# ShawnHuang497/MedPLIB

Measured on AMD Instinct MI355X. Metric: train samples/sec (img+64tok), higher is better.
Workload: dtype bf16

## Files before the change

### medplib_amd/csrc/gemm320_bf16.hip

```cpp
#include "gemm_common.h"
#include <stdlib.h>
#include <algorithm>

namespace {

constexpr int BM3 = 320, BN3 = 256, BK3 = 64, NT3 = 512;
constexpr int A_BYTES = BM3 * 128, B_BYTES = BN3 * 128, STAGE3 = A_BYTES + B_BYTES;

__device__ __forceinline__ int lds_off3(int r, int c) { return r * 128 + ((c ^ (r & 7)) << 4); }

#define MP3_BAR()                          \
  do {                                     \
    asm volatile("" ::: "memory");         \
    __builtin_amdgcn_sched_barrier(0);     \
    __builtin_amdgcn_s_barrier();          \
    __builtin_amdgcn_sched_barrier(0);     \
    asm volatile("" ::: "memory");         \
  } while (0)
#define MP3_LGKM0() asm volatile("s_waitcnt lgkmcnt(0)" ::: "memory")

constexpr int EPI_PLAIN = 0, EPI_ROPE = 1, EPI_SWIGLU = 2, EPI_COMBINE = 3, EPI_RELU = 4, EPI_GELU = 5;
template <int EPI>
__device__ __forceinline__ void gemm320_epilogue(const GemmArgs& g, f32x4 (&acc)[5][8], int batch, int M, int N, int m0, int n0, int wr, int wc,
                                                 int fr, int fq, unsigned items = 0xfffffu) {
  bf16_t* Cb = reinterpret_cast<bf16_t*>(g.C) + batch * g.sC;
  const int cw = n0 + wc * 128;
  const int c8 = pair_col8(fq);
  if constexpr (EPI == EPI_SWIGLU) {
    float rsc[5] = {1.f, 1.f, 1.f, 1.f, 1.f};
    if (g.a_scale) {
#pragma unroll
      for (int i = 0; i < 5; ++i) {
        const int row = m0 + wr * 80 + i * 16 + fr;
        if (row < M) rsc[i] = g.a_scale[g.a_rows ? g.a_rows[batch * g.rows_stride + row] : row];
      }
    }
#pragma unroll
    for (int i = 0; i < 5; ++i) {
      const int row = m0 + wr * 80 + i * 16 + fr;
#pragma unroll
      for (int jb = 0; jb < 2; ++jb) {
        if (!((items >> (i * 4 + jb * 2)) & 1u)) continue;
        bf16x4 o[2];
#pragma unroll
        for (int jj = 0; jj < 2; ++jj)
#pragma unroll
          for (int r = 0; r < 4; ++r) {
            acc[i][jb * 4 + jj][r] *= rsc[i];
            acc[i][jb * 4 + jj + 2][r] *= rsc[i];
            const float gf = (float)(bf16_t)acc[i][jb * 4 + jj][r];
            const float uf = (float)(bf16_t)acc[i][jb * 4 + jj + 2][r];
            o[jj][r] = (bf16_t)(gf * mp_sigmoid_fast(gf) * uf);
          }
        const bf16x8 p = pair_swap16(o[0], o[1]);
        if (row < M) *reinterpret_cast<bf16x8*>(Cb + (int64_t)row * g.ldc + (cw >> 1) + jb * 32 + c8) = p;
        if (g.keep_gu) {
          const bf16x8 pg = pair_swap16(round4(acc[i][jb * 4]), round4(acc[i][jb * 4 + 1])), pu = pair_swap16(round4(acc[i][jb * 4 + 2]), round4(acc[i][jb * 4 + 3]));
          if (row < M) {
            *reinterpret_cast<bf16x8*>(g.keep_gu + (int64_t)row * g.ld_gu + cw + jb * 64 + c8) = pg;
            *reinterpret_cast<bf16x8*>(g.keep_gu + (int64_t)row * g.ld_gu + cw + jb * 64 + 32 + c8) = pu;
          }
        }
      }
      __builtin_amdgcn_sched_barrier(0);
    }
    return;
  }
  if constexpr (EPI == EPI_COMBINE) {
    bf16_t* Cs = reinterpret_cast<bf16_t*>(g.C);
    int orow[5];
    float sc[5];
#pragma unroll
    for (int i = 0; i < 5; ++i) {
      const int row = m0 + wr * 80 + i * 16 + fr;
      orow[i] = row < M ? g.c_rows[batch * g.rows_stride + row] : -1;
    }
#pragma unroll
    for (int i = 0; i < 5; ++i) sc[i] = (orow[i] >= 0 && g.c_scale) ? g.c_scale[orow[i]] : 1.f;
#pragma unroll
    for (int h = 0; h < 2; ++h) {
      bf16x8 rv[5][2];
#pragma unroll
      for (int i = 0; i < 5; ++i)
#pragma unroll
        for (int jp = 0; jp < 2; ++jp) {
          const int col = cw + (h * 2 + jp) * 32 + c8;
          rv[i][jp] = bf16x8{};
          if (g.residual && orow[i] >= 0 && ((items >> (i * 4 + h * 2 + jp)) & 1u))
            rv[i][jp] = *reinterpret_cast<const bf16x8*>(g.residual + (int64_t)orow[i] * g.ldr + col);
        }
      __builtin_amdgcn_sched_barrier(0);
#pragma unroll
      for (int i = 0; i < 5; ++i)
#pragma unroll
        for (int jp = 0; jp < 2; ++jp) {
          const int col = cw + (h * 2 + jp) * 32 + c8;
          const bf16x8 p = pair_swap16(round4(acc[i][(h * 2 + jp) * 2]), round4(acc[i][(h * 2 + jp) * 2 + 1]));
          bf16x8 o;
#pragma unroll
          for (int e = 0; e < 8; ++e) {
            float v = (float)p[e] * sc[i];
            if (g.residual) v += (float)rv[i][jp][e];
            o[e] = (bf16_t)v;
          }
          if (orow[i] >= 0 && ((items >> (i * 4 + h * 2 + jp)) & 1u)) *reinterpret_cast<bf16x8*>(Cs + (int64_t)orow[i] * g.ldc + col) = o;
        }
      __builtin_amdgcn_sched_barrier(0);
    }
    return;
  }
  if constexpr (EPI == EPI_ROPE) {
    const bool is_v = n0 >= (N / 3) * 2;
    const int head0 = (cw >> 7) << 7;
    f32x4 cs[2][2][2], sn[2][2][2];
    float rsc[2] = {1.f, 1.f};
    auto fetch = [&](int i, int buf) {
      const int row = m0 + wr * 80 + i * 16 + fr;
      const int pos = (row < M ? row : 0) % g.rope_seq + g.rope_pos0;
      if (g.a_scale) rsc[buf] = g.a_scale[row < M ? row : 0];
#pragma unroll
      for (int jb = 0; jb < 2; ++jb)
#pragma unroll
        for (int jj = 0; jj < 2; ++jj) {
          const int dim = jb * 32 + jj * 16 + fq * 4;
          cs[buf][jb][jj] = *reinterpret_cast<const f32x4*>(g.rope_cos + (int64_t)pos * 64 + dim);
          sn[buf][jb][jj] = *reinterpret_cast<const f32x4*>(g.rope_sin + (int64_t)pos * 64 + dim);
        }
    };
    fetch(0, 0);
#pragma unroll
    for (int i = 0; i < 5; ++i) {
      if (i + 1 < 5) fetch(i + 1, (i + 1) & 1);
      __builtin_amdgcn_sched_barrier(0);
      const int row = m0 + wr * 80 + i * 16 + fr;
#pragma unroll
      for (int jb = 0; jb < 2; ++jb) {
        bf16x4 olo[2], ohi[2];
#pragma unroll
        for (int jj = 0; jj < 2; ++jj) {
          const bf16x4 qa = round4(acc[i][jb * 4 + jj] * rsc[i & 1]), qb = round4(acc[i][jb * 4 + jj + 2] * rsc[i & 1]);
#pragma unroll
          for (int r = 0; r < 4; ++r) {
            const float a = (float)qa[r], b = (float)qb[r];
            const bf16_t rlo = (bf16_t)(a * cs[i & 1][jb][jj][r] - b * sn[i & 1][jb][jj][r]);
            const bf16_t rhi = (bf16_t)(b * cs[i & 1][jb][jj][r] + a * sn[i & 1][jb][jj][r]);
            olo[jj][r] = is_v ? qa[r] : rlo;
            ohi[jj][r] = is_v ? qb[r] : rhi;
          }
        }
        const bf16x8 plo = pair_swap16(olo[0], olo[1]), phi = pair_swap16(ohi[0], ohi[1]);
        const int col_lo = (is_v ? cw + jb * 64 : head0 + jb * 32) + c8;
        const int col_hi = (is_v ? cw + jb * 64 + 32 : head0 + 64 + jb * 32) + c8;
        if (row < M) {
          *reinterpret_cast<bf16x8*>(Cb + (int64_t)row * g.ldc + col_lo) = plo;
          *reinterpret_cast<bf16x8*>(Cb + (int64_t)row * g.ldc + col_hi) = phi;
        }
      }
      __builtin_amdgcn_sched_barrier(0);
    }
    return;
  }
  const float* bias0 = g.bias ? g.bias + batch * g.sBias : nullptr;
  if (g.alpha != 1.f || bias0) {
#pragma unroll
    for (int j = 0; j < 8; ++j) {
      f32x4 bv = {0.f, 0.f, 0.f, 0.f};
      if (bias0) {
#pragma unroll
        for (int r = 0; r < 4; ++r) { const int col = cw + j * 16 + fq * 4 + r; bv[r] = col < N ? bias0[col] : 0.f; }
      }
#pragma unroll
      for (int i = 0; i < 5; ++i) acc[i][j] = acc[i][j] * g.alpha + bv;
    }
  }
#define MP3_ACT_SWEEP(EXPR)                                                          \
  _Pragma("unroll") for (int i = 0; i < 5; ++i) _Pragma("unroll") for (int j = 0; j < 8; ++j) {                    \
    _Pragma("unroll") for (int r = 0; r < 4; ++r) { const float v = acc[i][j][r]; acc[i][j][r] = (EXPR); }         \
    __builtin_amdgcn_sched_barrier(0);                                                                             \
  }
  if constexpr (EPI == EPI_RELU) { MP3_ACT_SWEEP(fmaxf(v, 0.f)) }
  else if constexpr (EPI == EPI_GELU) { MP3_ACT_SWEEP(gelu_erf_fast(v)) }
  else if (g.act == ACT_QUICK_GELU) { MP3_ACT_SWEEP(v * mp_sigmoid_fast(v, 1.702f)) }
#undef MP3_ACT_SWEEP
  const bf16_t* R = g.residual ? g.residual + batch * g.sR : nullptr;
#pragma unroll
  for (int h = 0; h < 2; ++h) {
    bf16x8 rv[5][2];
    if (R) {
#pragma unroll
      for (int i = 0; i < 5; ++i) {
        const int row = m0 + wr * 80 + i * 16 + fr;
#pragma unroll
        for (int jp = 0; jp < 2; ++jp) {
          const int col = cw + (h * 2 + jp) * 32 + c8;
          rv[i][jp] = bf16x8{};
          if (row < M && col < N && ((items >> (i * 4 + h * 2 + jp)) & 1u)) rv[i][jp] = *reinterpret_cast<const bf16x8*>(R + (int64_t)row * g.ldr + col);
        }
      }
      __builtin_amdgcn_sched_barrier(0);
    }
#pragma unroll
    for (int i = 0; i < 5; ++i) {
      const int row = m0 + wr * 80 + i * 16 + fr;
#pragma unroll
      for (int jp = 0; jp < 2; ++jp) {
        const int col = cw + (h * 2 + jp) * 32 + c8;
        bf16x8 p = pair_swap16(round4(acc[i][(h * 2 + jp) * 2]), round4(acc[i][(h * 2 + jp) * 2 + 1]));
        if (R) {
#pragma unroll
          for (int e = 0; e < 8; ++e) p[e] = (bf16_t)((float)p[e] + (float)rv[i][jp][e]);
        }
        if (row < M && col < N && ((items >> (i * 4 + h * 2 + jp)) & 1u)) *reinterpret_cast<bf16x8*>(Cb + (int64_t)row * g.ldc + col) = p;
      }
    }
    __builtin_amdgcn_sched_barrier(0);
  }
}

constexpr int MAX_FLAT_BATCH3 = 8;
template <int EPI>
__global__ __launch_bounds__(NT3, 1) void gemm320_bf16_nt_kernel(GemmArgs g) {
  extern __shared__ __attribute__((aligned(16))) char smem[];
  const int N = g.N;
  const int tiles_n = N / BN3;
  int T = 0;
  int pre[MAX_FLAT_BATCH3];
#pragma unroll
  for (int b = 0; b < MAX_FLAT_BATCH3; ++b) {
    pre[b] = T;
    if (b < g.nbatch) {
      const int Mb = g.m_dev ? min(g.M, g.m_dev[b * g.m_dev_stride]) : g.M;
      T += ((Mb + BM3 - 1) / BM3) * tiles_n;
    }
  }
  const int C = g.n_cu;
  const int full = (T / C) * C, rem = T - full;
  const int nt_all = g.K / BK3;
  int S = 1;
  if (g.ws && rem > 0 && rem * 2 <= C) S = max(1, min(min(min(C / rem, g.max_split), nt_all / 4), EPI == EPI_SWIGLU ? 10 : 20));
  const int bid = blockIdx.x;
  if (bid >= full + rem * S) return;
  int flat, split = 0;
  if (bid < full) {
    flat = (bid & 7) * (full >> 3) + (bid >> 3);
  } else {
    const int r = bid - full;
    if (S == 1 && (rem & 7) == 0) {
      flat = full + (r & 7) * (rem >> 3) + (r >> 3);
    } else {
      flat = full + r % rem;
      split = r / rem;
    }
  }
  const bool is_split = (bid >= full) && S > 1;
  int batch = 0, pbase = 0;
#pragma unroll
  for (int b = 1; b < MAX_FLAT_BATCH3; ++b) if (b < g.nbatch && flat >= pre[b]) { batch = b; pbase = pre[b]; }
  const int lid = flat - pbase;
  const int M = g.m_dev ? min(g.M, g.m_dev[batch * g.m_dev_stride]) : g.M;
  const int tiles_m = (M + BM3 - 1) / BM3;
  const int GROUP_M = g.group_m;
  const int per_group = GROUP_M * tiles_n;
  const int grp = lid / per_group;
  const int first_m = grp * GROUP_M;
  const int gsz = min(tiles_m - first_m, GROUP_M);
  const int tm = first_m + (lid % per_group) % gsz, tn = (lid % per_group) / gsz;
  const int m0 = tm * BM3, n0 = tn * BN3;
  int kt0 = 0, nt = nt_all;
  if (is_split) {
    const int base = nt_all / S, extra = nt_all % S;
    kt0 = split * base + min(split, extra);
    nt = base + (split < extra ? 1 : 0);
  }
  const int k_byte0 = kt0 * (BK3 * 2);

  const int tid = threadIdx.x;
  const int lane = tid & 63;
  const int wave = __builtin_amdgcn_readfirstlane(tid >> 6);
  const int wc = wave >> 2, wr = wave & 3;
  const int fr = lane & 15, fq = lane >> 4;

  const int sub_row = lane >> 3;
  const int src_c = (lane & 7) ^ sub_row;
  const __amdgpu_buffer_rsrc_t rs_a = __builtin_amdgcn_make_buffer_rsrc(const_cast<bf16_t*>(g.A + batch * g.sA), 0,
                                          g.a_rows ? 0x7ffffff0 : (int)(((int64_t)(M - 1) * g.lda + g.K) * 2), 0x00020000);
  const __amdgpu_buffer_rsrc_t rs_w = __builtin_amdgcn_make_buffer_rsrc(const_cast<bf16_t*>(g.W + batch * g.sW), 0, (int)(((int64_t)(N - 1) * g.ldw + g.K) * 2), 0x00020000);
  const int w_lane = (int)((sub_row * g.ldw + src_c * 8) * 2);
  const int w_row_bytes = (int)(g.ldw * 2);
  int a_off[5];
#pragma unroll
  for (int i = 0; i < 5; ++i) {
    int row = m0 + (wave + 8 * i) * 8 + sub_row;
    if (g.a_rows) row = g.a_rows[batch * g.rows_stride + min(row, M - 1)];
    a_off[i] = (int)(((int64_t)row * g.lda + src_c * 8) * 2);
  }
  int b_piece[4];
#pragma unroll
  for (int k = 0; k < 4; ++k) {
    const int e = 2 * wave + (k & 1);
    b_piece[k] = (e & 7) + (e >> 3) * 16 + (k >> 1) * 8;
  }
  auto dma_a = [&](int i, int t) {
    __builtin_amdgcn_raw_ptr_buffer_load_lds(rs_a, (__attribute__((address_space(3))) void*)(smem + (t & 1) * STAGE3 + (wave + 8 * i) * 1024), 16,
                                             a_off[i], k_byte0 + t * (BK3 * 2), 0, 0);
  };
  auto dma_b = [&](int k, int t) {
    __builtin_amdgcn_raw_ptr_buffer_load_lds(rs_w, (__attribute__((address_space(3))) void*)(smem + (t & 1) * STAGE3 + A_BYTES + b_piece[k] * 1024), 16,
                                             w_lane, (n0 + b_piece[k] * 8) * w_row_bytes + k_byte0 + t * (BK3 * 2), 0, 0);
  };

  f32x4 acc[5][8];
#pragma unroll
  for (int i = 0; i < 5; ++i)
#pragma unroll
    for (int j = 0; j < 8; ++j) acc[i][j] = f32x4{0.f, 0.f, 0.f, 0.f};
  bf16x8 fa[5][2], fb[4][2];
  const int a_rd0 = (wr * 80 + fr) * 128 + ((fq ^ (fr & 7)) << 4), a_rd1 = (wr * 80 + fr) * 128 + (((4 + fq) ^ (fr & 7)) << 4);
  const int b_rd0 = A_BYTES + (wc * 128 + fr) * 128 + ((fq ^ (fr & 7)) << 4), b_rd1 = A_BYTES + (wc * 128 + fr) * 128 + (((4 + fq) ^ (fr & 7)) << 4);
  auto load_a = [&](const char* st) {
#pragma unroll
    for (int i = 0; i < 5; ++i) {
      fa[i][0] = *reinterpret_cast<const bf16x8*>(st + a_rd0 + i * 2048);
      fa[i][1] = *reinterpret_cast<const bf16x8*>(st + a_rd1 + i * 2048);
    }
  };
  auto load_b = [&](int hn, const char* st) {
#pragma unroll
    for (int j = 0; j < 4; ++j) {
      fb[j][0] = *reinterpret_cast<const bf16x8*>(st + b_rd0 + (hn * 64 + j * 16) * 128);
      fb[j][1] = *reinterpret_cast<const bf16x8*>(st + b_rd1 + (hn * 64 + j * 16) * 128);
    }
  };
#ifndef MP3_PRIO
#define MP3_PRIO 0
#endif
#define MP3_MFMA_40(HN)                                                                                     \
  do {                                                                                                      \
    if (MP3_PRIO == 0) __builtin_amdgcn_s_setprio(1);                                                       \
    _Pragma("unroll") for (int kk = 0; kk < 2; ++kk)                                                        \
      _Pragma("unroll") for (int i = 0; i < 5; ++i)                                                         \
        _Pragma("unroll") for (int j = 0; j < 4; ++j)                                                       \
          acc[i][(HN) * 4 + j] = __builtin_amdgcn_mfma_f32_16x16x32_bf16(fb[j][kk], fa[i][kk], acc[i][(HN) * 4 + j], 0, 0, 0); \
    if (MP3_PRIO == 0) __builtin_amdgcn_s_setprio(0);                                                       \
    MP3_BAR();                                                                                              \
  } while (0)

#pragma unroll
  for (int i = 0; i < 5; ++i) dma_a(i, 0);
#pragma unroll
  for (int k = 0; k < 4; ++k) dma_b(k, 0);
  if (nt > 1) {
#pragma unroll
    for (int i = 0; i < 5; ++i) dma_a(i, 1);
    dma_b(0, 1); dma_b(1, 1);
    asm volatile("s_waitcnt vmcnt(7)" ::: "memory");
  } else {
    asm volatile("s_waitcnt vmcnt(0)" ::: "memory");
  }
  MP3_BAR();
  if (wc == 1) MP3_BAR();
  if (MP3_PRIO == 2 && wc == 1) __builtin_amdgcn_s_setprio(1);

  for (int t = 0; t < nt; ++t) {
    const char* st = smem + (t & 1) * STAGE3;
    const bool n1 = (t + 1 < nt), n2 = (t + 2 < nt);
    load_b(0, st);
    load_a(st);
    __builtin_amdgcn_sched_barrier(0);
    if (n1) { dma_b(2, t + 1); dma_b(3, t + 1); }
    MP3_LGKM0();
    MP3_BAR();
    MP3_MFMA_40(0);
    load_b(1, st);
    __builtin_amdgcn_sched_barrier(0);
    if (n2) {
#pragma unroll
      for (int i = 0; i < 5; ++i) dma_a(i, t + 2);
      dma_b(0, t + 2); dma_b(1, t + 2);
      asm volatile("s_waitcnt vmcnt(7)" ::: "memory");
    } else {
      asm volatile("s_waitcnt vmcnt(0)" ::: "memory");
    }
    MP3_LGKM0();
    MP3_BAR();
    MP3_MFMA_40(1);
  }
  if (wc == 0) MP3_BAR();
  if (MP3_PRIO == 2) __builtin_amdgcn_s_setprio(0);
  unsigned items = 0xfffffu;
  if (is_split) {
    typedef __attribute__((ext_vector_type(4))) unsigned int u32x4;
    constexpr int SLAB = BM3 * BN3 * 4;
    const int tail = flat - full;
    float* tile_ws = g.ws + ((int64_t)tail * S) * (BM3 * BN3);
    const __amdgpu_buffer_rsrc_t rs = __builtin_amdgcn_make_buffer_rsrc(tile_ws, 0, S * SLAB, 0x00020000);
    const int my_off = split * SLAB + tid * 16;
#pragma unroll
    for (int i = 0; i < 5; ++i)
#pragma unroll
      for (int j = 0; j < 8; ++j)
        __builtin_amdgcn_raw_buffer_store_b128(__builtin_bit_cast(u32x4, acc[i][j]), rs, my_off + (i * 8 + j) * (NT3 * 16), 0, 16);
    asm volatile("s_waitcnt vmcnt(0)" ::: "memory");
    __syncthreads();
    int* arrive = g.tickets + tail;
    int* depart = g.tickets + 128 + tail;
    int* mode = g.tickets + 256 + tail;
    constexpr int MODE_COOP = 1, MODE_LAST = 2;
    int* s_flag = reinterpret_cast<int*>(smem);
    if (tid == 0) {
      __hip_atomic_fetch_add(arrive, 1, __ATOMIC_RELAXED, __HIP_MEMORY_SCOPE_AGENT);
      const long long t0 = __builtin_amdgcn_s_memtime();
      int m = 0, seen = 0;
      for (;;) {
        seen = __hip_atomic_load(arrive, __ATOMIC_RELAXED, __HIP_MEMORY_SCOPE_AGENT);
        if (seen >= S) break;
        m = __hip_atomic_load(mode, __ATOMIC_RELAXED, __HIP_MEMORY_SCOPE_AGENT);
        if (m) break;
        if (__builtin_amdgcn_s_memtime() - t0 > g.tail_wait) break;
        __builtin_amdgcn_s_sleep(8);
      }
      if (!m) {
        int expected = 0;
        const int want = seen >= S ? MODE_COOP : MODE_LAST;
        m = __hip_atomic_compare_exchange_strong(mode, &expected, want, __ATOMIC_RELAXED, __ATOMIC_RELAXED, __HIP_MEMORY_SCOPE_AGENT) ? want : expected;
      }
      int last = 0;
      if (m == MODE_LAST) last = __hip_atomic_fetch_add(depart, 1, __ATOMIC_RELAXED, __HIP_MEMORY_SCOPE_AGENT) == S - 1;
      s_flag[0] = m | (last << 8);
    }
    __syncthreads();
    const int decided = s_flag[0];
    __syncthreads();
    const bool coop = (decided & 0xff) == MODE_COOP;
    if (!coop && !(decided >> 8)) return;
    constexpr int N_ITEMS = (EPI == EPI_SWIGLU) ? 10 : 20;
    items = 0;
#pragma unroll
    for (int it = 0; it < N_ITEMS; ++it)
      if (!coop || it % S == split) items |= (EPI == EPI_SWIGLU) ? (3u << (2 * it)) : (1u << it);
#pragma unroll
    for (int i = 0; i < 5; ++i)
#pragma unroll
      for (int j = 0; j < 8; ++j) acc[i][j] = f32x4{0.f, 0.f, 0.f, 0.f};
    for (int sp = 0; sp < S; ++sp) {
      const int base = sp * SLAB + tid * 16;
#pragma unroll
      for (int it = 0; it < 20; ++it) {
        if (!((items >> it) & 1u)) continue;
        const int i = it >> 2, j0 = (it & 3) * 2;
        u32x4 t[2];
#pragma unroll
        for (int q = 0; q < 2; ++q) t[q] = __builtin_amdgcn_raw_buffer_load_b128(rs, base + (i * 8 + j0 + q) * (NT3 * 16), 0, 16);
#pragma unroll
        for (int q = 0; q < 2; ++q) acc[i][j0 + q] += __builtin_bit_cast(f32x4, t[q]);
      }
    }
    asm volatile("s_waitcnt vmcnt(0)" ::: "memory");
    __syncthreads();
    if (tid == 0) {
      const bool rearm = coop ? (__hip_atomic_fetch_add(depart, 1, __ATOMIC_RELAXED, __HIP_MEMORY_SCOPE_AGENT) == S - 1) : true;
      if (rearm) {
        __hip_atomic_store(depart, 0, __ATOMIC_RELAXED, __HIP_MEMORY_SCOPE_AGENT);
        __hip_atomic_store(mode, 0, __ATOMIC_RELAXED, __HIP_MEMORY_SCOPE_AGENT);
        __hip_atomic_store(arrive, 0, __ATOMIC_RELAXED, __HIP_MEMORY_SCOPE_AGENT);
      }
    }
  }
  int tid2 = threadIdx.x;
  asm volatile("" : "+v"(tid2));
  gemm320_epilogue<EPI>(g, acc, batch, M, N, m0, n0, (tid2 >> 6) & 3, tid2 >> 8, tid2 & 15, (tid2 >> 4) & 3, items);
}

}

bool mp_gemm320_eligible(const GemmArgs& g, int batch) {
  if (batch < 1 || batch > MAX_FLAT_BATCH3 || g.out_f32) return false;
  if (g.keep_gu && (batch != 1 || (g.ld_gu & 7) || (reinterpret_cast<uintptr_t>(g.keep_gu) & 15))) return false;
  if (!(g.act == ACT_NONE || g.act == ACT_QUICK_GELU || g.act == ACT_ROPE_QK || g.act == ACT_SWIGLU_PAIR || g.act == ACT_RELU || g.act == ACT_GELU)) return false;
  if ((g.act == ACT_RELU || g.act == ACT_GELU) && (g.c_rows || g.a_rows)) return false;
  if (g.act == ACT_ROPE_QK && (batch != 1 || g.m_dev || g.a_rows || g.c_rows)) return false;
  if (g.act == ACT_SWIGLU_PAIR && (g.c_rows || g.residual || g.bias || g.alpha != 1.f || ((g.N >> 1) & 7))) return false;
  if (g.c_rows && (g.act != ACT_NONE || g.bias || g.alpha != 1.f)) return false;
  if (g.a_scale && !(g.act == ACT_ROPE_QK || g.act == ACT_SWIGLU_PAIR)) return false;
  if (g.N % BN3 || g.K % BK3 || g.M < (mp_gemm_policy_whole_tiles() ? BM3 : 1024)) return false;
  if ((g.ldc & 7) || (reinterpret_cast<uintptr_t>(g.C) & 15) || (g.sC & 7)) return false;
  if (g.residual && ((g.ldr & 7) || (reinterpret_cast<uintptr_t>(g.residual) & 15) || (g.sR & 7))) return false;
  const int64_t a_rows_bound = g.a_rows ? (int64_t)batch * g.M * 4 : (int64_t)g.M + 320;
  if (a_rows_bound * g.lda * 2 >= (1ll << 31) || (int64_t)g.N * g.ldw * 2 >= (1ll << 31)) return false;
  return true;
}

int mp_gemm320_subwave_split(const GemmArgs& g, int batch) {
  static int on = -1;
  if (on < 0) { const char* e = getenv("MP_GEMM320_SUBWAVE"); on = (e && atoi(e) == 0) ? 0 : 1; }
  if (!on || batch != 1 || g.m_dev || g.act == ACT_ROPE_QK || g.M < 1024 || g.K < 8192) return 1;
  if (mp_gemm_policy_whole_tiles()) return 1;
  const int C = std::min(mp_device_cus(), 256);
  const int64_t tiles = (int64_t)mp_cdiv(g.M, BM3) * (g.N / BN3);
  if (tiles * 2 > C || tiles * 4 <= C) return 1;
  const int64_t S = std::min<int64_t>(C / tiles, g.K / BK3 / 4);
  if (S < 2 || S * tiles * 10 < (int64_t)C * 9) return 1;
  return (int)S;
}

int mp_launch_gemm320(const GemmArgs& g0, int batch, hipStream_t stream) {
  static bool attr = false;
  if (!attr) {
    (void)hipFuncSetAttribute((const void*)gemm320_bf16_nt_kernel<EPI_PLAIN>, hipFuncAttributeMaxDynamicSharedMemorySize, 2 * STAGE3);
    (void)hipFuncSetAttribute((const void*)gemm320_bf16_nt_kernel<EPI_ROPE>, hipFuncAttributeMaxDynamicSharedMemorySize, 2 * STAGE3);
    (void)hipFuncSetAttribute((const void*)gemm320_bf16_nt_kernel<EPI_SWIGLU>, hipFuncAttributeMaxDynamicSharedMemorySize, 2 * STAGE3);
    (void)hipFuncSetAttribute((const void*)gemm320_bf16_nt_kernel<EPI_COMBINE>, hipFuncAttributeMaxDynamicSharedMemorySize, 2 * STAGE3);
    (void)hipFuncSetAttribute((const void*)gemm320_bf16_nt_kernel<EPI_RELU>, hipFuncAttributeMaxDynamicSharedMemorySize, 2 * STAGE3);
    (void)hipFuncSetAttribute((const void*)gemm320_bf16_nt_kernel<EPI_GELU>, hipFuncAttributeMaxDynamicSharedMemorySize, 2 * STAGE3);
    attr = true;
  }
  GemmArgs g = g0;
  g.nbatch = batch;
  g.n_cu = std::min(mp_device_cus(), 256);
  static int max_split = -1;
  if (max_split < 0) { const char* e = getenv("MP_GEMM320_MAX_SPLIT"); max_split = (e && atoi(e) >= 1) ? atoi(e) : 10; }
  static int dense_split = -1;
  if (dense_split < 0) { const char* e = getenv("MP_GEMM320_DENSE_SPLIT"); dense_split = (e && atoi(e) == 0) ? 0 : 1; }
  const int64_t dense_tiles = (int64_t)mp_cdiv(g.M, BM3) * (g.N / BN3);
  g.max_split = (batch > 1 || g.m_dev) ? max_split : ((dense_split && (dense_tiles > g.n_cu || mp_gemm320_subwave_split(g, batch) > 1)) ? max_split : 1);
  if (g.act == ACT_ROPE_QK) g.max_split = 1;
  if (mp_gemm_stream_registered(stream) || mp_gemm_policy_whole_tiles()) g.max_split = 1;
  g.tail_wait = mp_gemm_tail_wait_value();
  int64_t ws_bytes = 0;
  mp_gemm_split_workspace(stream, &g.ws, &g.tickets, &ws_bytes);
  if (!g.ws || ws_bytes < (int64_t)g.n_cu * BM3 * BN3 * 4) { g.ws = nullptr; g.tickets = nullptr; g.max_split = 1; }
  const int64_t host_tiles = (int64_t)mp_cdiv(g.M, BM3) * (g.N / BN3) * batch;
  const int64_t host_rem = host_tiles % g.n_cu;
  const bool may_split = g.max_split > 1 && (g.m_dev || (host_rem > 0 && host_rem * 2 <= g.n_cu));
  const dim3 grid((unsigned)(host_tiles + (may_split ? g.n_cu : 0)));
#define MP3_GO(E) hipLaunchKernelGGL(gemm320_bf16_nt_kernel<E>, grid, dim3(NT3), 2 * STAGE3, stream, g)
  if (g.act == ACT_ROPE_QK) MP3_GO(EPI_ROPE);
  else if (g.act == ACT_SWIGLU_PAIR) MP3_GO(EPI_SWIGLU);
  else if (g.c_rows) MP3_GO(EPI_COMBINE);
  else if (g.act == ACT_RELU) MP3_GO(EPI_RELU);
  else if (g.act == ACT_GELU) MP3_GO(EPI_GELU);
  else MP3_GO(EPI_PLAIN);
#undef MP3_GO
  return mp_check_launch("mp_gemm_bf16_nt(320)");
}
```

Before: 138.5.

## Skip MFMA and epilogue work for padded rows in partial M tiles

Changes the per-wave row mapping of the 320-row tile from contiguous 80-row blocks to 16-row fragments interleaved across waves, so that a partial last M tile leaves whole fragments empty. Each wave counts its live fragments and dispatches a K loop specialised at compile time on that count, skipping LDS reads and MFMAs for rows beyond M. Epilogue and split-K workspace writes are masked the same way, and gathered A rows past M now fall outside the buffer range instead of reading a clamped row. This adds six instantiations of the K loop, which grows code size and may raise register pressure, and it only helps shapes whose M is not a multiple of 320.

```diff
diff --git a/medplib_amd/csrc/gemm320_bf16.hip b/medplib_amd/csrc/gemm320_bf16.hip
--- a/medplib_amd/csrc/gemm320_bf16.hip
+++ b/medplib_amd/csrc/gemm320_bf16.hip
@@ -1,13 +1,18 @@
 #include "gemm_common.h"
 #include <stdlib.h>
 #include <algorithm>
+#include <type_traits>
 
 namespace {
 
 constexpr int BM3 = 320, BN3 = 256, BK3 = 64, NT3 = 512;
 constexpr int A_BYTES = BM3 * 128, B_BYTES = BN3 * 128, STAGE3 = A_BYTES + B_BYTES;
+constexpr int A_GATHER_RANGE = 0x7ffffff0;
 
 __device__ __forceinline__ int lds_off3(int r, int c) { return r * 128 + ((c ^ (r & 7)) << 4); }
+
+__device__ __forceinline__ int frag_row3(int wr, int i) { return (wr + 4 * i) * 16; }
+__device__ __forceinline__ int live_frag_rows3(int R, int wr) { return max(0, min(5, (((min(R, BM3) + 15) >> 4) - wr + 3) >> 2)); }
 
 #define MP3_BAR()                          \
   do {                                     \
@@ -31,13 +36,13 @@
     if (g.a_scale) {
 #pragma unroll
       for (int i = 0; i < 5; ++i) {
-        const int row = m0 + wr * 80 + i * 16 + fr;
+        const int row = m0 + frag_row3(wr, i) + fr;
         if (row < M) rsc[i] = g.a_scale[g.a_rows ? g.a_rows[batch * g.rows_stride + row] : row];
       }
     }
 #pragma unroll
     for (int i = 0; i < 5; ++i) {
-      const int row = m0 + wr * 80 + i * 16 + fr;
+      const int row = m0 + frag_row3(wr, i) + fr;
 #pragma unroll
       for (int jb = 0; jb < 2; ++jb) {
         if (!((items >> (i * 4 + jb * 2)) & 1u)) continue;
@@ -72,7 +77,7 @@
     float sc[5];
 #pragma unroll
     for (int i = 0; i < 5; ++i) {
-      const int row = m0 + wr * 80 + i * 16 + fr;
+      const int row = m0 + frag_row3(wr, i) + fr;
       orow[i] = row < M ? g.c_rows[batch * g.rows_stride + row] : -1;
     }
 #pragma unroll
@@ -94,6 +99,7 @@
       for (int i = 0; i < 5; ++i)
 #pragma unroll
         for (int jp = 0; jp < 2; ++jp) {
+          if (!((items >> (i * 4 + h * 2 + jp)) & 1u)) continue;
           const int col = cw + (h * 2 + jp) * 32 + c8;
           const bf16x8 p = pair_swap16(round4(acc[i][(h * 2 + jp) * 2]), round4(acc[i][(h * 2 + jp) * 2 + 1]));
           bf16x8 o;
@@ -103,7 +109,7 @@
             if (g.residual) v += (float)rv[i][jp][e];
             o[e] = (bf16_t)v;
           }
-          if (orow[i] >= 0 && ((items >> (i * 4 + h * 2 + jp)) & 1u)) *reinterpret_cast<bf16x8*>(Cs + (int64_t)orow[i] * g.ldc + col) = o;
+          if (orow[i] >= 0) *reinterpret_cast<bf16x8*>(Cs + (int64_t)orow[i] * g.ldc + col) = o;
         }
       __builtin_amdgcn_sched_barrier(0);
     }
@@ -115,7 +121,7 @@
     f32x4 cs[2][2][2], sn[2][2][2];
     float rsc[2] = {1.f, 1.f};
     auto fetch = [&](int i, int buf) {
-      const int row = m0 + wr * 80 + i * 16 + fr;
+      const int row = m0 + frag_row3(wr, i) + fr;
       const int pos = (row < M ? row : 0) % g.rope_seq + g.rope_pos0;
       if (g.a_scale) rsc[buf] = g.a_scale[row < M ? row : 0];
 #pragma unroll
@@ -132,7 +138,8 @@
     for (int i = 0; i < 5; ++i) {
       if (i + 1 < 5) fetch(i + 1, (i + 1) & 1);
       __builtin_amdgcn_sched_barrier(0);
-      const int row = m0 + wr * 80 + i * 16 + fr;
+      const int row = m0 + frag_row3(wr, i) + fr;
+      if (!((items >> (i * 4)) & 1u)) continue;
 #pragma unroll
       for (int jb = 0; jb < 2; ++jb) {
         bf16x4 olo[2], ohi[2];
@@ -189,7 +196,7 @@
     if (R) {
 #pragma unroll
       for (int i = 0; i < 5; ++i) {
-        const int row = m0 + wr * 80 + i * 16 + fr;
+        const int row = m0 + frag_row3(wr, i) + fr;
 #pragma unroll
         for (int jp = 0; jp < 2; ++jp) {
           const int col = cw + (h * 2 + jp) * 32 + c8;
@@ -201,16 +208,17 @@
     }
 #pragma unroll
     for (int i = 0; i < 5; ++i) {
-      const int row = m0 + wr * 80 + i * 16 + fr;
+      const int row = m0 + frag_row3(wr, i) + fr;
 #pragma unroll
       for (int jp = 0; jp < 2; ++jp) {
+        if (!((items >> (i * 4 + h * 2 + jp)) & 1u)) continue;
         const int col = cw + (h * 2 + jp) * 32 + c8;
         bf16x8 p = pair_swap16(round4(acc[i][(h * 2 + jp) * 2]), round4(acc[i][(h * 2 + jp) * 2 + 1]));
         if (R) {
 #pragma unroll
           for (int e = 0; e < 8; ++e) p[e] = (bf16_t)((float)p[e] + (float)rv[i][jp][e]);
         }
-        if (row < M && col < N && ((items >> (i * 4 + h * 2 + jp)) & 1u)) *reinterpret_cast<bf16x8*>(Cb + (int64_t)row * g.ldc + col) = p;
+        if (row < M && col < N) *reinterpret_cast<bf16x8*>(Cb + (int64_t)row * g.ldc + col) = p;
       }
     }
     __builtin_amdgcn_sched_barrier(0);
@@ -283,7 +291,7 @@
   const int sub_row = lane >> 3;
   const int src_c = (lane & 7) ^ sub_row;
   const __amdgpu_buffer_rsrc_t rs_a = __builtin_amdgcn_make_buffer_rsrc(const_cast<bf16_t*>(g.A + batch * g.sA), 0,
-                                          g.a_rows ? 0x7ffffff0 : (int)(((int64_t)(M - 1) * g.lda + g.K) * 2), 0x00020000);
+                                          g.a_rows ? A_GATHER_RANGE : (int)(((int64_t)(M - 1) * g.lda + g.K) * 2), 0x00020000);
   const __amdgpu_buffer_rsrc_t rs_w = __builtin_amdgcn_make_buffer_rsrc(const_cast<bf16_t*>(g.W + batch * g.sW), 0, (int)(((int64_t)(N - 1) * g.ldw + g.K) * 2), 0x00020000);
   const int w_lane = (int)((sub_row * g.ldw + src_c * 8) * 2);
   const int w_row_bytes = (int)(g.ldw * 2);
@@ -291,8 +299,9 @@
 #pragma unroll
   for (int i = 0; i < 5; ++i) {
     int row = m0 + (wave + 8 * i) * 8 + sub_row;
-    if (g.a_rows) row = g.a_rows[batch * g.rows_stride + min(row, M - 1)];
-    a_off[i] = (int)(((int64_t)row * g.lda + src_c * 8) * 2);
+    const bool absent = g.a_rows && row >= M;
+    if (g.a_rows && !absent) row = g.a_rows[batch * g.rows_stride + row];
+    a_off[i] = absent ? A_GATHER_RANGE : (int)(((int64_t)row * g.lda + src_c * 8) * 2);
   }
   int b_piece[4];
 #pragma unroll
@@ -315,13 +324,13 @@
 #pragma unroll
     for (int j = 0; j < 8; ++j) acc[i][j] = f32x4{0.f, 0.f, 0.f, 0.f};
   bf16x8 fa[5][2], fb[4][2];
-  const int a_rd0 = (wr * 80 + fr) * 128 + ((fq ^ (fr & 7)) << 4), a_rd1 = (wr * 80 + fr) * 128 + (((4 + fq) ^ (fr & 7)) << 4);
+  const int a_rd0 = (wr * 16 + fr) * 128 + ((fq ^ (fr & 7)) << 4), a_rd1 = (wr * 16 + fr) * 128 + (((4 + fq) ^ (fr & 7)) << 4);
   const int b_rd0 = A_BYTES + (wc * 128 + fr) * 128 + ((fq ^ (fr & 7)) << 4), b_rd1 = A_BYTES + (wc * 128 + fr) * 128 + (((4 + fq) ^ (fr & 7)) << 4);
-  auto load_a = [&](const char* st) {
-#pragma unroll
-    for (int i = 0; i < 5; ++i) {
-      fa[i][0] = *reinterpret_cast<const bf16x8*>(st + a_rd0 + i * 2048);
-      fa[i][1] = *reinterpret_cast<const bf16x8*>(st + a_rd1 + i * 2048);
+  auto load_a = [&](const char* st, auto ni_c) {
+#pragma unroll
+    for (int i = 0; i < decltype(ni_c)::value; ++i) {
+      fa[i][0] = *reinterpret_cast<const bf16x8*>(st + a_rd0 + frag_row3(0, i) * 128);
+      fa[i][1] = *reinterpret_cast<const bf16x8*>(st + a_rd1 + frag_row3(0, i) * 128);
     }
   };
   auto load_b = [&](int hn, const char* st) {
@@ -338,7 +347,7 @@
   do {                                                                                                      \
     if (MP3_PRIO == 0) __builtin_amdgcn_s_setprio(1);                                                       \
     _Pragma("unroll") for (int kk = 0; kk < 2; ++kk)                                                        \
-      _Pragma("unroll") for (int i = 0; i < 5; ++i)                                                         \
+      _Pragma("unroll") for (int i = 0; i < NI; ++i)                                                        \
         _Pragma("unroll") for (int j = 0; j < 4; ++j)                                                       \
           acc[i][(HN) * 4 + j] = __builtin_amdgcn_mfma_f32_16x16x32_bf16(fb[j][kk], fa[i][kk], acc[i][(HN) * 4 + j], 0, 0, 0); \
     if (MP3_PRIO == 0) __builtin_amdgcn_s_setprio(0);                                                       \
@@ -361,17 +370,20 @@
   if (wc == 1) MP3_BAR();
   if (MP3_PRIO == 2 && wc == 1) __builtin_amdgcn_s_setprio(1);
 
+  const int ni = live_frag_rows3(M - m0, wr);
+  auto k_loop = [&](auto ni_c) {
+  constexpr int NI = decltype(ni_c)::value;
   for (int t = 0; t < nt; ++t) {
     const char* st = smem + (t & 1) * STAGE3;
     const bool n1 = (t + 1 < nt), n2 = (t + 2 < nt);
-    load_b(0, st);
-    load_a(st);
+    if constexpr (NI > 0) load_b(0, st);
+    load_a(st, ni_c);
     __builtin_amdgcn_sched_barrier(0);
     if (n1) { dma_b(2, t + 1); dma_b(3, t + 1); }
     MP3_LGKM0();
     MP3_BAR();
     MP3_MFMA_40(0);
-    load_b(1, st);
+    if constexpr (NI > 0) load_b(1, st);
     __builtin_amdgcn_sched_barrier(0);
     if (n2) {
 #pragma unroll
@@ -385,9 +397,19 @@
     MP3_BAR();
     MP3_MFMA_40(1);
   }
+  };
+  switch (ni) {
+    case 5: k_loop(std::integral_constant<int, 5>{}); break;
+    case 4: k_loop(std::integral_constant<int, 4>{}); break;
+    case 3: k_loop(std::integral_constant<int, 3>{}); break;
+    case 2: k_loop(std::integral_constant<int, 2>{}); break;
+    case 1: k_loop(std::integral_constant<int, 1>{}); break;
+    default: k_loop(std::integral_constant<int, 0>{}); break;
+  }
   if (wc == 0) MP3_BAR();
   if (MP3_PRIO == 2) __builtin_amdgcn_s_setprio(0);
-  unsigned items = 0xfffffu;
+  const unsigned live = (1u << (4 * ni)) - 1u;
+  unsigned items = live;
   if (is_split) {
     typedef __attribute__((ext_vector_type(4))) unsigned int u32x4;
     constexpr int SLAB = BM3 * BN3 * 4;
@@ -396,10 +418,12 @@
     const __amdgpu_buffer_rsrc_t rs = __builtin_amdgcn_make_buffer_rsrc(tile_ws, 0, S * SLAB, 0x00020000);
     const int my_off = split * SLAB + tid * 16;
 #pragma unroll
-    for (int i = 0; i < 5; ++i)
+    for (int i = 0; i < 5; ++i) {
+      if (i >= ni) continue;
 #pragma unroll
       for (int j = 0; j < 8; ++j)
         __builtin_amdgcn_raw_buffer_store_b128(__builtin_bit_cast(u32x4, acc[i][j]), rs, my_off + (i * 8 + j) * (NT3 * 16), 0, 16);
+    }
     asm volatile("s_waitcnt vmcnt(0)" ::: "memory");
     __syncthreads();
     int* arrive = g.tickets + tail;
@@ -438,6 +462,7 @@
 #pragma unroll
     for (int it = 0; it < N_ITEMS; ++it)
       if (!coop || it % S == split) items |= (EPI == EPI_SWIGLU) ? (3u << (2 * it)) : (1u << it);
+    items &= live;
 #pragma unroll
     for (int i = 0; i < 5; ++i)
 #pragma unroll
```

Result: no change. 138.9, median of 6 (+0.3%).
